# Wu-sm/Adversarial-Attacks-on-GAN-based-Image-Fusion

Measured on AMD Instinct MI355X. Metric: attacked images/sec, PGD-20 L∞ ε=8/255 at 256², 1/2/4/8 MI355X, higher is better.
Workload: dtype f32; 1 GPU; PGD-20 L∞ eps=8/255 alpha=2/255 at 256², 128 images/GPU (BASELINE config #4 per-GPU share), RCCL all-gather of outputs when N>1; encoder=e4e, norm=linf, images_per_gpu=128, global_batch=128, size=256, pgd_steps=20, parallelism=dp1, dist_world_size=1, output_in_eps_ball_and_finite=True, fp32_arithmetic=fp32

## Files before the change

adversarial-attacks-on-gan-based-image-fusion_amd/csrc/conv_halo_x6.hip:

```cpp
#include <type_traits>

#include "conv_common.h"
#include "halo_epilogue.h"

namespace mia {

#ifdef MIA_STAMPS
__device__ unsigned long long g_x6_stamps[4][24];
#endif

template <int BN_, int TPS_ = 1>
struct HaloX6 {
  static constexpr int PH = 16, PW = 16, NW = 8, NT = 64 * NW;
  static constexpr int WN = BN_ == 128 ? 2 : 1, WM = NW / WN, FM = 16 / WM, FN = 4;
  static constexpr int BM = PH * PW, BN = BN_, BK = 32;
  static constexpr int HSIDE = PW + 2, HROWS = (PH + 2) * HSIDE;
  static constexpr int HPIECES = (HROWS + 7) / 8;
  static constexpr int HBUF = HPIECES * 1024;
  static constexpr int LROWB = 64, LBUF = HROWS * LROWB;
  static constexpr int TPS = TPS_, NG = (9 + TPS - 1) / TPS;
  static constexpr int BHM = BN * ROWB, BL = BN * LROWB, BSTAGE1 = BHM + BL;
  static constexpr int BSTAGE = TPS * BSTAGE1;
  static constexpr int BWAVES = 4, HWAVES = 4;
  static constexpr int B_HM_INS = BN / 8 / BWAVES;
// ... 480 lines not shown
    atomicAdd(g + 6, (unsigned long long)nk);
    atomicAdd(g + 7, st_wb);
  }
  if (wid == 4 && lane == 0) atomicAdd(&g_x6_stamps[(BN_ == 128 ? 1 : 0) + (PRO ? 2 : 0)][8], st_wb);
  if ((wid == 0 || wid == 4) && lane == 0) {
    unsigned long long* g = g_x6_stamps[(BN_ == 128 ? 1 : 0) + (PRO ? 2 : 0)] + (wid ? 13 : 9);
    atomicAdd(g + 0, st_rd);
    atomicAdd(g + 1, st_m0);
    atomicAdd(g + 2, st_arr);
    atomicAdd(g + 3, st_rel);
  }
#endif
}

template <int BN_, bool PRO, int EPI, bool EARLY, bool PRIO = false, bool UNR = false,
          int TPS = 1, int STG = 0>
static int launch_x6_e(ConvK& k, hipStream_t st) {
  MIA_CONV_PATH("halo_x6", EPI);
  typedef HaloX6<BN_, TPS> TL;
  k.nbn = (k.a.Cout + TL::BN - 1) / TL::BN;
  k.nblk = k.a.N * (k.a.H / TL::PH) * (k.a.W / TL::PW) * k.nbn;
  size_t lds = TL::LDS;
  lds = std::max(lds, (size_t)TL::EROWS * TL::ES * 4);
  lds = std::max(lds, (size_t)TL::NW * TL::BN * 4);
  auto fn = conv_halo_x6_kernel<BN_, PRO, EPI, EARLY, PRIO, UNR, TPS, STG>;
  if (const int rc = ensure_dyn_lds((const void*)fn, 160 * 1024); rc != MIA_OK) return rc;
  k.prered = EPI >= 0 && (EPI & epi::CSUM);
  const int H = k.a.H, W = k.a.W;
  const int nslots = EPI >= 0    ? halo_red_slots(H, W, TL::FM, TL::WM, k.prered)
                     : EPI == -1 ? halo_red_slots(H, W, TL::FM, TL::WM, false)
                                 : (H / TL::PH) * (W / TL::PW);
  RedQ r;
  int rc = conv_red_begin(k, r, nslots, st);
  if (rc != MIA_OK) return rc;
  hipLaunchKernelGGL(fn, dim3(k.nblk), dim3(TL::NT), lds, st, k);
  rc = check_launch("conv_halo_x6");
  return rc != MIA_OK ? rc : red_finish(r, st);
}

constexpr bool x6_stagger_wins(bool pro, int epi) {
#ifdef MIA_X6_STAGGER_ALL
  return MIA_X6_STAGGER_ALL != 0;
#else
  (void)epi;
  return !pro;
#endif
}

template <int BN_, bool PRO, int EPI>
static int launch_x6_(ConvK& k, hipStream_t st) {
  if constexpr (EPI >= 0) {
    const int u = tune(T_X6_UNR);
    if constexpr (BN_ == 64) {
      if (u == 2) return launch_x6_e<BN_, PRO, EPI, true, true, true, 2>(k, st);
    }
    if constexpr (BN_ == 128) {
      const int sg = tune(T_X6_STAGGER);
      if (u != 0 && (sg < 0 ? x6_stagger_wins(PRO, EPI) : sg != 0))
        return launch_x6_e<BN_, PRO, EPI, true, true, true, 1, 1>(k, st);
    }
    if (u != 0) return launch_x6_e<BN_, PRO, EPI, true, true, true>(k, st);
  }
  return launch_x6_e<BN_, PRO, EPI, true, true>(k, st);
}

struct HaloX6S {
  static constexpr int PH = 8, PW = 16, NW = 4, NT = 64 * NW;
  static constexpr int WN = 1, WM = 4, FM = 2, FN = 4;
  static constexpr int BM = PH * PW, BN = 64, BK = 32;
  static constexpr int HSIDE = PW + 2, HROWS = (PH + 2) * HSIDE;
  static constexpr int HPIECES = (HROWS + 7) / 8;
  static constexpr int HBUF = HPIECES * 1024;
  static constexpr int LROWB = 64, LBUF = HROWS * LROWB;
  static constexpr int BHM = BN * ROWB, BL = BN * LROWB, BSTAGE = BHM + BL;
  static constexpr int B_HM_INS = BN / 8 / NW, B_L_INS = BN / 16 / NW;
  static constexpr int H_INS = (HPIECES + NW - 1) / NW;
  static constexpr int EROWS = 128, ES = BN + 4;
  static constexpr int LDS = HBUF + LBUF + 2 * BSTAGE;
  static_assert(WM * FM * 16 == BM && WN * FN * 16 == BN, "");
  static_assert(B_HM_INS * 8 * NW == BN && B_L_INS * 16 * NW == BN, "");
  static_assert(LDS <= 80 * 1024, "two blocks per CU");
};

template <bool PRO, int EPI>
__global__ __launch_bounds__(HaloX6S::NT, 2) void conv_halo_x6s_kernel(const ConvK k) {
  static_assert(EPI >= 0, "the specialised register epilogues only");
  typedef HaloX6S TL;
  constexpr int FM = TL::FM, FN = TL::FN, NT = TL::NT, BN = TL::BN, BK = TL::BK;
  constexpr int HSIDE = TL::HSIDE, HROWS = TL::HROWS, HPIECES = TL::HPIECES;
  constexpr int H_INS = TL::H_INS, B_HM_INS = TL::B_HM_INS, B_L_INS = TL::B_L_INS;
  constexpr int BSTAGE = TL::BSTAGE;

  extern __shared__ __attribute__((aligned(16))) char smem[];
  char* const hbuf = smem;
  char* const lbuf = smem + TL::HBUF;
  char* const bring = lbuf + TL::LBUF;

  const mia_conv_args& p = k.a;
  const int tid = threadIdx.x, lane = tid & 63;
  const int wid = __builtin_amdgcn_readfirstlane(tid >> 6);
  const int wm = wid, wn = 0;
  const ConvGroup G = k.g[0];
  const int H = p.H, W = p.W, Cin = p.Cin, Cout = p.Cout, Kpad = G.kpad;
  const int bl = xcd_remap(blockIdx.x, k.nblk);
  const int mt = bl / k.nbn, n0 = (bl % k.nbn) * BN;
  const int ptx = W / TL::PW, pty = H / TL::PH;
  const int x0 = (mt % ptx) * TL::PW;
  const int y0 = ((mt / ptx) % pty) * TL::PH;
  const int n = mt / (ptx * pty);

  const float* __restrict__ X = (const float*)p.x;
  const unsigned* __restrict__ Whm = (const unsigned*)G.w_split;
  const __bf16* __restrict__ Wl = (const __bf16*)(Whm + (size_t)Cout * Kpad);
  const char* zero = (const char*)g_zero16;

  const char* wsrc[B_HM_INS + B_L_INS];
#pragma unroll
  for (int j = 0; j < B_HM_INS + B_L_INS; ++j) {
    if (j < B_HM_INS) {
      const int row = (wid * B_HM_INS + j) * 8 + (lane >> 3);
      const int c = min(n0 + row, Cout - 1);
      wsrc[j] = (const char*)(Whm + (size_t)c * Kpad + ((lane & 7) ^ fsw(row)) * 4);
    } else {
      const int row = (wid * B_L_INS + j - B_HM_INS) * 16 + (lane >> 2);
      const int c = min(n0 + row, Cout - 1);
      wsrc[j] = (const char*)(Wl + (size_t)c * Kpad + ((lane & 3) ^ (lsw(row) >> 1)) * 8);
    }
  }
  const char* hsrc[H_INS];
#pragma unroll
  for (int j = 0; j < H_INS; ++j) {
    hsrc[j] = nullptr;
    const int hr = (wid + TL::NW * j) * 8 + (lane >> 3);
    const int hy = hr / HSIDE, hx = hr - (hr / HSIDE) * HSIDE;
    const int y = y0 + hy - 1, x = x0 + hx - 1;
    if (hr < HROWS && y >= 0 && y < H && x >= 0 && x < W)
      hsrc[j] = (const char*)(X + ((size_t)(n * H + y) * W + x) * Cin + ((lane & 7) ^ fsw(hr)) * 4);
  }
  const int ncb = Cin / BK, nk = 9 * ncb;

  auto issue_b = [&](int s, int st) {
    const int cb = s / 9, t = s - (s / 9) * 9;
    const size_t koff = (size_t)t * Cin + cb * BK;
    char* dst = bring + st * BSTAGE;
#pragma unroll
    for (int j = 0; j < B_HM_INS; ++j)
      __builtin_amdgcn_global_load_lds((gptr_t)(wsrc[j] + koff * 4),
                                       (lptr_t)(dst + (wid * B_HM_INS + j) * 1024), 16, 0, 0);
#pragma unroll
    for (int j = 0; j < B_L_INS; ++j)
      __builtin_amdgcn_global_load_lds((gptr_t)(wsrc[B_HM_INS + j] + koff * 2),
                                       (lptr_t)(dst + TL::BHM + (wid * B_L_INS + j) * 1024), 16,
                                       0, 0);
  };
  auto issue_halo = [&](int cb) {
#pragma unroll
    for (int j = 0; j < H_INS; ++j) {
      if (wid + TL::NW * j >= HPIECES) break;
      const char* a = hsrc[j] ? hsrc[j] + (size_t)cb * BK * 4 : zero;
      __builtin_amdgcn_global_load_lds((gptr_t)a, (lptr_t)(hbuf + (wid + TL::NW * j) * 1024), 16,
                                       0, 0);
    }
  };
  const bool lrelu_in = p.act_in == MIA_ACT_LRELU_S2;
  auto convert = [&](int cb) {
    for (int c = tid; c < HROWS * 8; c += NT) {
      const int hr = c >> 3, pc = c & 7, lc = pc ^ fsw(hr);
      f32x4 v = *(const f32x4*)(hbuf + hr * ROWB + pc * 16);
      if constexpr (PRO) {
        const float mul = lrelu_in ? SQRT2 : 1.f;
        f32x4 s4 = {1.f, 1.f, 1.f, 1.f};
        if (p.in_scale) s4 = *(const f32x4*)(p.in_scale + (size_t)n * Cin + cb * BK + lc * 4);
#pragma unroll
        for (int e = 0; e < 4; ++e) {
          float f = v[e];
          if (lrelu_in) f = fmaxf(f, 0.2f * f);
          v[e] = f * (s4[e] * mul);
        }
      }
      u32x4 hm;
      u32x2 lo;
      split_quad(v, hm, lo);
      *(u32x4*)(hbuf + hr * ROWB + pc * 16) = hm;
      *(u32x2*)(lbuf + hr * TL::LROWB + ((lc ^ lsw(hr)) << 3)) = lo;
    }
  };

  issue_halo(0);
  issue_b(0, 0);
  asm volatile("s_waitcnt vmcnt(0)" ::: "memory");
  __syncthreads();
  convert(0);
  __syncthreads();

  f32x4 acc[FM][FN];
#pragma unroll
  for (int i = 0; i < FM; ++i)
#pragma unroll
    for (int j = 0; j < FN; ++j) acc[i][j] = f32x4{0.f, 0.f, 0.f, 0.f};

  const int frow = lane & 15, fq = lane >> 4;
  int oh[FM + 2][3], ol[FM + 2][3];
#pragma unroll
  for (int q = 0; q < FM + 2; ++q)
#pragma unroll
    for (int c = 0; c < 3; ++c) {
      const int hr = (wm * FM + q) * HSIDE + frow + c;
      int vh = hr * ROWB + ((fq ^ fsw(hr)) << 4), vl = hr * TL::LROWB + ((fq ^ lsw(hr)) << 3);
      asm volatile("" : "+v"(vh), "+v"(vl));
      oh[q][c] = vh;
      ol[q][c] = vl;
    }
  int st = 0;
  for (int cb = 0; cb < ncb; ++cb) {
#pragma unroll
    for (int t = 0; t < 9; ++t) {
      const int s = cb * 9 + t;
      int x1 = 64, x2 = 32;
      asm volatile("" : "+s"(x1), "+s"(x2));
      const int dy = t / 3, dx = t % 3;
      const char* sb = bring + st * BSTAGE;
      if (s + 1 < nk) issue_b(s + 1, st ^ 1);
#pragma unroll
      for (int h = 0; h < 2; ++h) {
        const int ch = h * 4 + fq;
        u32x4 ahm[FM], bhm[FN];
        u32x2 al[FM], blo[FN];
#pragma unroll
        for (int i = 0; i < FM; ++i) {
          ahm[i] = *(const u32x4*)(hbuf + (h ? oh[i + dy][dx] ^ x1 : oh[i + dy][dx]));
          al[i] = *(const u32x2*)(lbuf + (h ? ol[i + dy][dx] ^ x2 : ol[i + dy][dx]));
        }
#pragma unroll
        for (int j = 0; j < FN; ++j) {
          const int row = 16 * j + frow;
          bhm[j] = *(const u32x4*)(sb + row * ROWB + ((ch ^ fsw(row)) << 4));
          blo[j] = *(const u32x2*)(sb + TL::BHM + row * TL::LROWB + ((ch ^ lsw(row)) << 3));
        }
        __builtin_amdgcn_s_setprio(1);
#pragma unroll
        for (int i = 0; i < FM; ++i)
#pragma unroll
          for (int j = 0; j < FN; ++j)
            acc[i][j] = mfma_x6(bhm[j], blo[j], ahm[i], al[i], acc[i][j]);
        __builtin_amdgcn_s_setprio(0);
      }
      asm volatile("s_waitcnt vmcnt(0)" ::: "memory");
      lds_handoff();
      __builtin_amdgcn_sched_barrier(0);
      st ^= 1;
    }
    if (cb + 1 < ncb) {
      issue_halo(cb + 1);
      asm volatile("s_waitcnt vmcnt(0)" ::: "memory");
      __syncthreads();
      convert(cb + 1);
      __syncthreads();
    }
  }
  halo_epilogue_f<float, TL, EPI>(k, acc, n, y0, x0, n0, wm, wn, lane, -1, -1, nullptr,
                                  k.prered ? (float*)smem : nullptr, TL::WM, TL::BN);
}

template <bool PRO, int EPI>
static int launch_x6s_(ConvK& k, hipStream_t st) {
  MIA_CONV_PATH("halo_x6", EPI);
  typedef HaloX6S TL;
  k.nbn = (k.a.Cout + TL::BN - 1) / TL::BN;
  k.nblk = k.a.N * (k.a.H / TL::PH) * (k.a.W / TL::PW) * k.nbn;
  size_t lds = TL::LDS;
  lds = std::max(lds, (size_t)TL::EROWS * TL::ES * 4);
  lds = std::max(lds, (size_t)TL::NW * TL::BN * 4);
  auto fn = conv_halo_x6s_kernel<PRO, EPI>;
  if (const int rc = ensure_dyn_lds((const void*)fn, 80 * 1024); rc != MIA_OK) return rc;
  k.prered = (EPI & epi::CSUM);
  const int nslots = halo_red_slots(k.a.H, k.a.W, TL::FM, TL::WM, k.prered);
  RedQ r;
  int rc = conv_red_begin(k, r, nslots, st);
  if (rc != MIA_OK) return rc;
  hipLaunchKernelGGL(fn, dim3(k.nblk), dim3(TL::NT), lds, st, k);
  rc = check_launch("conv_halo_x6s");
  return rc != MIA_OK ? rc : red_finish(r, st);
}

constexpr int X6S_NONE = 1;
static int launch_x6s(ConvK& k, hipStream_t st, bool pro) {
  using namespace epi;
  const int f = epi_mask(k);
  if (pro) {
    if (f == (OSC | NOISE | BIAS | LRELU)) return launch_x6s_<true, OSC | NOISE | BIAS | LRELU>(k, st);
    return X6S_NONE;
  }
  switch (f) {
    case 0: return launch_x6s_<false, 0>(k, st);
    case BIAS: return launch_x6s_<false, BIAS>(k, st);
    case BIAS | RELU: return launch_x6s_<false, BIAS | RELU>(k, st);
    case PRELU: return launch_x6s_<false, PRELU>(k, st);
    case MASK: return launch_x6s_<false, MASK>(k, st);
    case TAP: return launch_x6s_<false, TAP>(k, st);
    case TAP | MASK: return launch_x6s_<false, TAP | MASK>(k, st);
    case ACC: return launch_x6s_<false, ACC>(k, st);
    case MASK | MSL: return launch_x6s_<false, MASK | MSL>(k, st);
    default: return X6S_NONE;
  }
}

template <int BN_, bool PRO>
static int launch_x6_spec(ConvK& k, hipStream_t st) {
  using namespace epi;
  const int f = epi_mask(k);
  if constexpr (PRO) {
    if (f == (OSC | NOISE | BIAS | LRELU))
      return launch_x6_<BN_, PRO, OSC | NOISE | BIAS | LRELU>(k, st);
  } else if constexpr (BN_ == 64) {
    switch (f) {
      case 0: return launch_x6_<BN_, PRO, 0>(k, st);
      case BIAS: return launch_x6_<BN_, PRO, BIAS>(k, st);
      case BIAS | RELU: return launch_x6_<BN_, PRO, BIAS | RELU>(k, st);
      case PRELU: return launch_x6_<BN_, PRO, PRELU>(k, st);
      case MASK: return launch_x6_<BN_, PRO, MASK>(k, st);
      case TAP: return launch_x6_<BN_, PRO, TAP>(k, st);
      case ACC: return launch_x6_<BN_, PRO, ACC>(k, st);
      case MASK | MSL: return launch_x6_<BN_, PRO, MASK | MSL>(k, st);
      default: break;
    }
  } else {
    switch (f) {
      case 0: return launch_x6_<BN_, PRO, 0>(k, st);
      case BIAS: return launch_x6_<BN_, PRO, BIAS>(k, st);
      case BIAS | RELU: return launch_x6_<BN_, PRO, BIAS | RELU>(k, st);
      case PRELU: return launch_x6_<BN_, PRO, PRELU>(k, st);
      case MASK: return launch_x6_<BN_, PRO, MASK>(k, st);
      case TAP: return launch_x6_<BN_, PRO, TAP>(k, st);
      case ACC: return launch_x6_<BN_, PRO, ACC>(k, st);
      case MASK | MSL: return launch_x6_<BN_, PRO, MASK | MSL>(k, st);
      case OSC | SDOT: return launch_x6_<BN_, PRO, OSC | SDOT>(k, st);
      case OSC | SDOT | BAB: return launch_x6_<BN_, PRO, OSC | SDOT | BAB>(k, st);
      default: break;
    }
  }
  return launch_x6_<BN_, PRO, -1>(k, st);
}

bool conv_halo_x6_eligible(const ConvK& k, int dtype) {
#ifdef MIA_F32_NATIVE
  (void)k;
  (void)dtype;
  return false;
#endif
  if (tune(T_CONV_X6) == 0) return false;
  const mia_conv_args& a = k.a;
  const ConvGroup& G = k.g[0];
  return dtype == MIA_F32 && G.w_split != nullptr && k.ng == 1 && k.stride == 1 && G.kh == 3 &&
         G.kw == 3 && G.pad_y == 1 && G.pad_x == 1 && G.ho == a.H && G.wo == a.W && G.ay == 1 &&
         G.ax == 1 && G.by == 0 && G.bx == 0 && !a.shuffle_out && a.H % 16 == 0 &&
         a.W % 16 == 0 && a.Cin % 32 == 0 && k.HT == a.H && k.WT == a.W &&
         a.Cout >= 64;
}

#ifdef MIA_STAMPS
extern "C" int mia_debug_x6_stamps(unsigned long long* host, int reset) {
  if (hipMemcpyFromSymbol(host, HIP_SYMBOL(g_x6_stamps), sizeof(g_x6_stamps)) != hipSuccess)
    return 1;
  if (reset) {
    static const unsigned long long zero[4][24] = {};
// ... 39 lines not shown
```

adversarial-attacks-on-gan-based-image-fusion_amd/csrc/conv_upconv.hip:

```cpp
#include "conv_common.h"

namespace mia {

template <int BN_>
struct HaloUpT {
  static constexpr int PH = 8, PW = 16, NW = 4, NT = 256;
  static constexpr int WN = BN_ == 64 ? 2 : 1, WM = NW / WN, FM = PH / WM, FN = 2;
  static constexpr int BN = WN * FN * 16;
  static constexpr int HSIDE = PW + 1, HROWS = (PH + 1) * HSIDE;
  static constexpr int HPIECES = (HROWS + 7) / 8;
  static constexpr int HBUF = HPIECES * 8 * ROWB;
  static constexpr int BROWS = 2 * BN, BSTAGE = BROWS * ROWB;
  static constexpr int BWAVES = 2, HWAVES = 2;
  static constexpr int B_INS = BROWS / (8 * BWAVES);
  static constexpr int H_INS = (HPIECES + HWAVES - 1) / HWAVES;
  static constexpr int HPS = (H_INS + 3) / 4;
  static constexpr int NSTEP = 5, STAGES = 2;
  static_assert(B_INS * 8 * BWAVES == BROWS && H_INS * HWAVES == HPIECES, "");
  static_assert(WM * FM == PH && WN * FN * 16 == BN_, "");
};
typedef HaloUpT<64> HaloUp;

__device__ __forceinline__ constexpr int up_jy(int st) { return st == 3 || st == 4 ? 1 : 0; }
__device__ __forceinline__ constexpr int up_jx(int st) { return st == 2 || st == 4 ? 1 : 0; }
// ... 537 lines not shown
#pragma unroll
            for (int j = 0; j < FN; ++j)
              acc[ph][i][j] = mfma_x6(bhm[j], blo[j], ahm[i], al[i], acc[ph][i][j]);
          if constexpr (PRIO) __builtin_amdgcn_s_setprio(0);
        }
        if (!EARLY && h == 0 && !bwave && st < 4 && cb + 1 < ncb) {
          __builtin_amdgcn_sched_barrier(0);
#pragma unroll
          for (int q = 0; q < HPS; ++q) {
            const int j = st * HPS + q;
            if (j < H_INS && hw + HWAVES * j < HPIECES) issue_h(cb + 1, j, (cb + 1) & 1);
          }
          __builtin_amdgcn_sched_barrier(0);
        }
      }
      if (bwave || st == TL::NSTEP - 1) asm volatile("s_waitcnt vmcnt(0)" ::: "memory");
      __builtin_amdgcn_s_waitcnt(0xc07f);
      __builtin_amdgcn_s_barrier();
      __builtin_amdgcn_sched_barrier(0);
      if (st == TL::NSTEP - 1 && cb + 1 < ncb) {
        convert(cb + 1);
        __syncthreads();
      }
    }
  }

  const int frow = lane & 15, fq = lane >> 4;
  float* __restrict__ Y = (float*)k.t;
  const int TS = DG ? 2 * R : 2 * R + 1;
  float msl[FN][4];
#pragma unroll
  for (int j = 0; j < FN; ++j)
#pragma unroll
    for (int e = 0; e < 4; ++e)
      msl[j][e] = k.mask_slope ? k.mask_slope[n0 + wn * FN * 16 + 16 * j + 4 * fq + e] : 0.f;
#pragma unroll
  for (int ph = 0; ph < 4; ++ph) {
    const int py = ph >> 1, px = ph & 1;
#pragma unroll
    for (int i = 0; i < FM; ++i) {
      const int ty = 2 * (y0 + wm * FM + i) + (DG ? 1 - py : py);
      const int tx = 2 * (x0 + frow) + (DG ? 1 - px : px);
#pragma unroll
      for (int j = 0; j < FN; ++j) {
        const int c = n0 + wn * FN * 16 + 16 * j + 4 * fq;
        const size_t o = ((size_t)(n * TS + ty) * TS + tx) * Cout + c;
        f32x4 v = acc[ph][i][j];
        if (DG && k.mask_a) {
          const f32x4 m = *(const f32x4*)((const float*)k.mask_a + o);
#pragma unroll
          for (int e = 0; e < 4; ++e) v[e] = m[e] > 0.f ? v[e] : msl[j][e] * v[e];
        }
        if (DG && k.accumulate) {
          const f32x4 a = *(const f32x4*)(Y + o);
#pragma unroll
          for (int e = 0; e < 4; ++e) v[e] += a[e];
        }
        *(f32x4*)(Y + o) = v;
      }
    }
  }
}

struct DgX6S {
  static constexpr int PH = 8, PW = 16, NW = 4, NT = 64 * NW;
  static constexpr int WM = 4, WN = 1, FM = 2, FN = 4;
  static constexpr int BN = WN * FN * 16, BK = 32;
  static constexpr int HSIDE = PW + 1, HROWS = (PH + 1) * HSIDE;
  static constexpr int HPIECES = (HROWS + 7) / 8;
  static constexpr int HBUF = HPIECES * 1024;
  static constexpr int LROWB = 64, LBUF = HROWS * LROWB;
  static constexpr int BROWS = 2 * BN;
  static constexpr int BHM = BROWS * ROWB, BSTAGE = BHM + BROWS * LROWB;
  static constexpr int B_HM_INS = BROWS / 8 / NW;
  static constexpr int B_L_INS = BROWS / 16 / NW;
  static constexpr int H_INS = (HPIECES + NW - 1) / NW;
  static constexpr int NSTEP = 5;
  static constexpr int LDS = HBUF + LBUF + 2 * BSTAGE;
  static_assert(WM * FM == PH && WN * FN * 16 == BN, "");
  static_assert(B_HM_INS * 8 * NW == BROWS && B_L_INS * 16 * NW == BROWS, "");
  static_assert(LDS <= 80 * 1024, "two blocks per CU");
};

template <bool DG, bool PRO>
__global__ __launch_bounds__(DgX6S::NT, 2) void upconv_x6s_kernel(const UpK k) {
  typedef DgX6S TL;
  constexpr int FM = TL::FM, FN = TL::FN, WN = TL::WN, BN = TL::BN, BK = TL::BK, NT = TL::NT;
  constexpr int HSIDE = TL::HSIDE, HROWS = TL::HROWS, HPIECES = TL::HPIECES;
  constexpr int H_INS = TL::H_INS, BSTAGE = TL::BSTAGE;
  constexpr int B_HM_INS = TL::B_HM_INS, B_L_INS = TL::B_L_INS;

  extern __shared__ __attribute__((aligned(16))) char smem[];
  char* const hbuf = smem;
  char* const lbuf = smem + TL::HBUF;
  char* const bring = lbuf + TL::LBUF;

  const int tid = threadIdx.x, lane = tid & 63;
  const int wid = __builtin_amdgcn_readfirstlane(tid >> 6);
  const int wm = wid / WN, wn = wid % WN;
  const int R = k.R, Cin = k.Cin, Cout = k.Cout;
  const int bl = xcd_remap(blockIdx.x, k.nblk);
  const int mt = bl / k.nbn, n0 = (bl % k.nbn) * BN;
  const int ptx = R / TL::PW, pty = R / TL::PH;
  const int x0 = (mt % ptx) * TL::PW;
  const int y0 = ((mt / ptx) % pty) * TL::PH;
  const int n = mt / (ptx * pty);
  const int ncb = Cin / BK, nk = TL::NSTEP * ncb;
  const int csrc = k.cin_src, cbs = csrc / BK;
  const char* Whm = (const char*)k.w_split;
  const char* Wl = Whm + (size_t)nk * 2 * Cout * ROWB;
  const size_t hm_step = (size_t)2 * Cout * ROWB, l_step = (size_t)2 * Cout * TL::LROWB;
  const char* zero = (const char*)g_zero16;

  int woff[B_HM_INS + B_L_INS], hoff[H_INS];
#pragma unroll
  for (int j = 0; j < B_HM_INS + B_L_INS; ++j) {
    if (j < B_HM_INS) {
      const int row = (wid * B_HM_INS + j) * 8 + (lane >> 3);
      const int slot = row / BN, c = n0 + row % BN;
      woff[j] = (slot * Cout + c) * ROWB + ((lane & 7) ^ fsw(row)) * 16;
    } else {
      const int row = (wid * B_L_INS + j - B_HM_INS) * 16 + (lane >> 2);
      const int slot = row / BN, c = n0 + row % BN;
      woff[j] = (slot * Cout + c) * TL::LROWB + ((lane & 3) ^ (lsw(row) >> 1)) * 16;
    }
  }
#pragma unroll
  for (int j = 0; j < H_INS; ++j) {
    hoff[j] = -1;
    const int hr = (wid + TL::NW * j) * 8 + (lane >> 3);
    const int hy = hr / HSIDE, hx = hr - (hr / HSIDE) * HSIDE;
    const int y = y0 + hy - (DG ? 0 : 1), x = x0 + hx - (DG ? 0 : 1);
    if (hr < HROWS && y >= 0 && y < R && x >= 0 && x < R)
      hoff[j] = ((n * R + y) * R + x) * csrc + ((lane & 7) ^ fsw(hr)) * 4;
  }
  auto opaque = [](int v) __attribute__((always_inline)) {
    asm volatile("" : "+v"(v));
    return v;
  };
  auto issue_b = [&](int s, int stg) {
    char* dst = bring + stg * BSTAGE;
    const char* hm = Whm + s * hm_step;
    const char* lo = Wl + s * l_step;
#pragma unroll
    for (int j = 0; j < B_HM_INS; ++j)
      __builtin_amdgcn_global_load_lds((gptr_t)(hm + opaque(woff[j])),
                                       (lptr_t)(dst + (wid * B_HM_INS + j) * 1024), 16, 0, 0);
#pragma unroll
    for (int j = 0; j < B_L_INS; ++j)
      __builtin_amdgcn_global_load_lds((gptr_t)(lo + opaque(woff[B_HM_INS + j])),
                                       (lptr_t)(dst + TL::BHM + (wid * B_L_INS + j) * 1024), 16,
                                       0, 0);
  };
  auto issue_halo = [&](int cb) {
    const int sc = cb / cbs;
    const float* xb = (const float*)up_src(k, sc) + (cb - sc * cbs) * BK;
#pragma unroll
    for (int j = 0; j < H_INS; ++j) {
      if (wid + TL::NW * j >= HPIECES) break;
      const int o = opaque(hoff[j]);
      const char* a = o >= 0 ? (const char*)(xb + o) : zero;
      __builtin_amdgcn_global_load_lds((gptr_t)a, (lptr_t)(hbuf + (wid + TL::NW * j) * 1024), 16,
                                       0, 0);
    }
  };
  const bool lrelu_in = k.act_in == MIA_ACT_LRELU_S2;
  auto convert = [&](int cb) {
    for (int c = tid; c < HROWS * 8; c += NT) {
      const int hr = c >> 3, pc = c & 7, lc = pc ^ fsw(hr);
      f32x4 v = *(const f32x4*)(hbuf + hr * ROWB + pc * 16);
      if constexpr (PRO) {
        const float mul = lrelu_in ? SQRT2 : 1.f;
        f32x4 s4 = {1.f, 1.f, 1.f, 1.f};
        if (k.style) s4 = *(const f32x4*)(k.style + (size_t)n * Cin + cb * BK + lc * 4);
#pragma unroll
        for (int e = 0; e < 4; ++e) {
          float f = v[e];
          if (lrelu_in) f = fmaxf(f, 0.2f * f);
          v[e] = f * (s4[e] * mul);
        }
      }
      u32x4 hm;
      u32x2 lo;
      split_quad(v, hm, lo);
      *(u32x4*)(hbuf + hr * ROWB + pc * 16) = hm;
      *(u32x2*)(lbuf + hr * TL::LROWB + ((lc ^ lsw(hr)) << 3)) = lo;
    }
  };

  issue_halo(0);
  issue_b(0, 0);
  asm volatile("s_waitcnt vmcnt(0)" ::: "memory");
  __syncthreads();
  convert(0);
  __syncthreads();

  f32x4 acc[4][FM][FN];
#pragma unroll
  for (int q = 0; q < 4; ++q)
#pragma unroll
    for (int i = 0; i < FM; ++i)
#pragma unroll
      for (int j = 0; j < FN; ++j) acc[q][i][j] = f32x4{0.f, 0.f, 0.f, 0.f};

  for (int cb = 0; cb < ncb; ++cb) {
#pragma unroll
    for (int st = 0; st < TL::NSTEP; ++st) {
      const int ln = opaque(lane);
      const int frow = ln & 15, fq = ln >> 4;
      const int s = cb * TL::NSTEP + st;
      const char* sb = bring + (s & 1) * BSTAGE;
      if (s + 1 < nk) issue_b(s + 1, (s & 1) ^ 1);
      const int jy = up_jy(st), jx = up_jx(st);
#pragma unroll
      for (int h = 0; h < 2; ++h) {
        const int ch = h * 4 + fq;
        u32x4 ahm[FM];
        u32x2 al[FM];
#pragma unroll
        for (int i = 0; i < FM; ++i) {
          const int hr = DG ? (wm * FM + i + jy) * HSIDE + frow + jx
                            : (wm * FM + i + 1 - jy) * HSIDE + frow + 1 - jx;
          ahm[i] = *(const u32x4*)(hbuf + hr * ROWB + ((ch ^ fsw(hr)) << 4));
          al[i] = *(const u32x2*)(lbuf + hr * TL::LROWB + ((ch ^ lsw(hr)) << 3));
        }
#pragma unroll
        for (int slot = 0; slot < 2; ++slot) {
          const int ph = up_phase(st, slot);
          if (ph < 0) continue;
          u32x4 bhm[FN];
          u32x2 blo[FN];
#pragma unroll
          for (int j = 0; j < FN; ++j) {
            const int row = slot * BN + wn * FN * 16 + 16 * j + frow;
            bhm[j] = *(const u32x4*)(sb + row * ROWB + ((ch ^ fsw(row)) << 4));
            blo[j] = *(const u32x2*)(sb + TL::BHM + row * TL::LROWB + ((ch ^ lsw(row)) << 3));
          }
#pragma unroll
          for (int i = 0; i < FM; ++i)
#pragma unroll
            for (int j = 0; j < FN; ++j)
              acc[ph][i][j] = mfma_x6(bhm[j], blo[j], ahm[i], al[i], acc[ph][i][j]);
        }
      }
      asm volatile("s_waitcnt vmcnt(0)" ::: "memory");
      lds_handoff();
      __builtin_amdgcn_sched_barrier(0);
    }
    if (cb + 1 < ncb) {
      issue_halo(cb + 1);
      asm volatile("s_waitcnt vmcnt(0)" ::: "memory");
      __syncthreads();
      convert(cb + 1);
      __syncthreads();
    }
  }

  const int frow = lane & 15, fq = lane >> 4;
  float* __restrict__ Y = (float*)k.t;
  const int TS = DG ? 2 * R : 2 * R + 1;
  float msl[FN][4];
#pragma unroll
  for (int j = 0; j < FN; ++j)
#pragma unroll
    for (int e = 0; e < 4; ++e)
      msl[j][e] = k.mask_slope ? k.mask_slope[n0 + wn * FN * 16 + 16 * j + 4 * fq + e] : 0.f;
#pragma unroll
  for (int ph = 0; ph < 4; ++ph) {
    const int py = ph >> 1, px = ph & 1;
#pragma unroll
    for (int i = 0; i < FM; ++i) {
      const int ty = 2 * (y0 + wm * FM + i) + (DG ? 1 - py : py);
      const int tx = 2 * (x0 + frow) + (DG ? 1 - px : px);
#pragma unroll
      for (int j = 0; j < FN; ++j) {
        const int c = n0 + wn * FN * 16 + 16 * j + 4 * fq;
        const size_t o = ((size_t)(n * TS + ty) * TS + tx) * Cout + c;
        f32x4 v = acc[ph][i][j];
        if (DG && k.mask_a) {
          const f32x4 m = *(const f32x4*)((const float*)k.mask_a + o);
#pragma unroll
          for (int e = 0; e < 4; ++e) v[e] = m[e] > 0.f ? v[e] : msl[j][e] * v[e];
        }
        if (DG && k.accumulate) {
          const f32x4 a = *(const f32x4*)(Y + o);
#pragma unroll
          for (int e = 0; e < 4; ++e) v[e] += a[e];
        }
        *(f32x4*)(Y + o) = v;
      }
    }
  }
}

template <bool DG, bool PRO>
static int launch_upconv_x6s(UpK& k, hipStream_t st) {
  typedef DgX6S TL;
  set_conv_path(DG ? "s2dg_x6s" : "upconv_x6s");
  k.nbn = k.Cout / TL::BN;
  k.nblk = k.N * (k.R / TL::PH) * (k.R / TL::PW) * k.nbn;
  auto fn = upconv_x6s_kernel<DG, PRO>;
  if (const int rc = ensure_dyn_lds((const void*)fn, 80 * 1024); rc != MIA_OK) return rc;
  hipLaunchKernelGGL(fn, dim3(k.nblk), dim3(TL::NT), TL::LDS, st, k);
  return check_launch("upconv_x6s");
}

template <bool DG, bool PRO, bool EARLY, bool PRIO>
static int launch_upconv_x6_e(UpK& k, hipStream_t st) {
  typedef DgX6 TL;
  set_conv_path(DG ? "s2dg_x6" : "upconv_x6");
  k.nbn = k.Cout / TL::BN;
  k.nblk = k.N * (k.R / TL::PH) * (k.R / TL::PW) * k.nbn;
  auto fn = upconv_x6_kernel<DG, PRO, EARLY, PRIO>;
  if (const int rc = ensure_dyn_lds((const void*)fn, 160 * 1024); rc != MIA_OK) return rc;
  hipLaunchKernelGGL(fn, dim3(k.nblk), dim3(TL::NT), TL::LDS, st, k);
  return check_launch("upconv_x6");
}

template <bool DG, bool PRO>
static int launch_upconv_x6(UpK& k, hipStream_t st) {
  if (DG && tune(T_UPCONV_X6S) != 0 && k.Cin <= 512) return launch_upconv_x6s<DG, PRO>(k, st);
  return launch_upconv_x6_e<DG, PRO, true, false>(k, st);
}

static bool upconv_x6_ok(const UpK& k, int dtype) {
#ifdef MIA_F32_NATIVE
  (void)k;
  (void)dtype;
  return false;
#else
  if (tune(T_UPCONV_X6) == 0) return false;
  return dtype == MIA_F32 && k.w_split && k.R % DgX6::PH == 0 && k.Cout % DgX6::BN == 0 &&
         k.Cin % DgX6::BK == 0;
#endif
}

static bool s2dg_x6_ok(const UpK& k, int dtype) {
#ifdef MIA_F32_NATIVE
  (void)k;
  (void)dtype;
  return false;
#else
  if (tune(T_S2DG_X6) == 0) return false;
  return dtype == MIA_F32 && k.w_split && k.R % DgX6::PH == 0 && k.Cout % DgX6::BN == 0 &&
         k.cin_src % DgX6::BK == 0;
#endif
}

bool s2_dgrad_halo_eligible(int dtype, int R, int Cg, int Cx) {
  if (tune(T_S2DG_HALO) == 0) return false;
  (void)dtype;
  return R % 16 == 0 && Cg % 64 == 0 && Cx % HaloUp::BN == 0 &&
         (int64_t)4 * R * R < (1LL << 31);
}

}

using namespace mia;

extern "C" int mia_conv_s2_dgrad_halo_multi(const void* const* g, int ng, const void* w_halo,
                                            const void* w_split, void* gx, int N, int R, int Cg,
                                            int Cx, const void* mask_a, const float* mask_slope,
                                            int accumulate, int dtype, void* stream) {
  MIA_CHECK_ARG(g && ng >= 1 && ng <= UP_MAX_SRC && w_halo && gx && N > 0, "bad args");
  for (int i = 0; i < ng; ++i) MIA_CHECK_ARG(g[i], "null source tensor");
  MIA_CHECK_ARG(s2_dgrad_halo_eligible(dtype, R, Cg, Cx),
                "needs R % 16 == 0, Cg % 64 == 0, Cx % 64 == 0 "
                "(use mia_conv2d phase groups otherwise)");
  MIA_CHECK_ARG((int64_t)N * R * R * Cg < (1LL << 31), "input too large for 32-bit offsets");
  UpK k = {};
  k.x = g[0]; k.w = w_halo; k.t = gx; k.mask_a = mask_a; k.mask_slope = mask_slope;
  k.N = N; k.R = R; k.Cin = ng * Cg; k.Cout = Cx; k.accumulate = accumulate;
  for (int i = 0; i < ng; ++i) k.xs[i] = g[i];
  k.cin_src = Cg;
  k.w_split = w_split;
  if (s2dg_x6_ok(k, dtype)) return launch_upconv_x6<true, false>(k, (hipStream_t)stream);
  MIA_DISPATCH_DTYPE(dtype, T, return launch_upconv_halo<T, false, true>(k, (hipStream_t)stream));
  return set_error("s2_dgrad_halo: unknown dtype");
}


extern "C" int mia_conv_s2_dgrad_halo(const void* g, const void* w_halo, void* gx, int N, int R,
                                      int Cg, int Cx, const void* mask_a, const float* mask_slope,
                                      int accumulate, int dtype, void* stream) {
  const void* gs[1] = {g};
  return mia_conv_s2_dgrad_halo_multi(gs, 1, w_halo, nullptr, gx, N, R, Cg, Cx, mask_a,
                                      mask_slope, accumulate, dtype, stream);
// ... 2 lines not shown
```

adversarial-attacks-on-gan-based-image-fusion_amd/csrc/mia_common.h:

```cpp
#pragma once
#include <hip/hip_runtime.h>
#include <stdint.h>
#include <string>

#include "../../include/miattack.h"

namespace mia {

typedef __attribute__((ext_vector_type(4))) float f32x4;
typedef __attribute__((ext_vector_type(8))) _Float16 f16x8;
typedef __attribute__((ext_vector_type(8))) __bf16 bf16x8;

template <typename T> struct Vec;
template <> struct Vec<float> { typedef f32x4 type; static constexpr int N = 4; };
template <> struct Vec<_Float16> { typedef f16x8 type; static constexpr int N = 8; };
template <> struct Vec<__bf16> { typedef bf16x8 type; static constexpr int N = 8; };

__device__ __forceinline__ float to_f(float v) { return v; }
__device__ __forceinline__ float to_f(_Float16 v) { return (float)v; }
__device__ __forceinline__ float to_f(__bf16 v) { return (float)v; }
template <typename T> __device__ __forceinline__ T from_f(float v);
template <> __device__ __forceinline__ float from_f<float>(float v) { return v; }
template <> __device__ __forceinline__ _Float16 from_f<_Float16>(float v) { return (_Float16)v; }
template <> __device__ __forceinline__ __bf16 from_f<__bf16>(float v) { return (__bf16)v; }

constexpr float SQRT2 = 1.41421356237309504880f;

__device__ __forceinline__ float lrelu_s2(float v) { return (v > 0.f ? v : 0.2f * v) * SQRT2; }
__device__ __forceinline__ float lrelu_s2_grad(float pre) { return pre > 0.f ? SQRT2 : 0.2f * SQRT2; }
__device__ __forceinline__ float lrelu_s2_inv_grad(float pre) {
  return pre > 0.f ? 0.70710678118654752f : 3.5355339059327376f;
}

#define MIA_DPP(v, ctrl) \
  __builtin_bit_cast(float, __builtin_amdgcn_mov_dpp(__builtin_bit_cast(int, (v)), (ctrl), 0xf, 0xf, false))
__device__ __forceinline__ void lds_handoff() {
  asm volatile("s_waitcnt lgkmcnt(0)\n\ts_barrier" ::: "memory");
}

__device__ __forceinline__ float row16_sum(float v) {
  v += MIA_DPP(v, 0xB1);
  v += MIA_DPP(v, 0x4E);
  v += MIA_DPP(v, 0x141);
  v += MIA_DPP(v, 0x140);
  return v;
}

__device__ __forceinline__ float wave_sum(float v) {
#pragma unroll
  for (int o = 32; o > 0; o >>= 1) v += __shfl_xor(v, o, 64);
  return v;
}

int set_error(const std::string& msg);
int check_launch(const char* what);

int device_cu_count();
int ensure_dyn_lds(const void* fn, int bytes);
int max_blocks_per_cu(const void* fn, int threads, size_t dyn_lds);

enum TuneKey {
  T_CONV_HALO,
  T_CONV_X6,
  T_HALO_EPI,
  T_X6_UNR,
  T_CONV_THIN,
  T_CONV_THIN32,
  T_CONV_WRES,
  T_CONV_REGEPI,
  T_CONV_SMALLTILE,
  T_S2DG_X6,
  T_S2DG_HALO,
  T_UPCONV_X6,
  T_UPCONV_HALO,
  T_CONV_WRES32,
  T_HALO_C64,
  T_X6_64S,
  T_UPCONV_X6S,
  T_CONV_WRES128,
  T_X6_STAGGER,
  T_NKEYS
};
int tune(TuneKey key);

struct RedQ {
  float* dst[3];
  float* part;
  int nslots, count;
};
float* red_scratch(hipStream_t st, size_t bytes);
int red_begin(RedQ& r, float* d0, float* d1, float* d2, int nslots, int count, hipStream_t st,
              bool zero = false);
int red_finish(const RedQ& r, hipStream_t st);

__device__ __forceinline__ void red_store(float* part, int nslots, int count, int q, int slot,
                                          int i, float v) {
  part[((size_t)q * nslots + slot) * count + i] = v;
}

}

#define MIA_DISPATCH_DTYPE(dtype, T, ...)                                   \
  switch (dtype) {                                                          \
    case MIA_F32: { typedef float T; __VA_ARGS__; break; }                  \
    case MIA_F16: { typedef _Float16 T; __VA_ARGS__; break; }               \
    case MIA_BF16: { typedef __bf16 T; __VA_ARGS__; break; }                \
    default: return mia::set_error("unsupported dtype");                    \
  }

#define MIA_CHECK_ARG(cond, msg) \
  do { if (!(cond)) return mia::set_error(std::string(__func__) + ": " + (msg)); } while (0)
```

adversarial-attacks-on-gan-based-image-fusion_amd/csrc/reduce.hip:

```cpp
#include <algorithm>
#include <cstdlib>
#include <cstring>
#include <mutex>
#include <unordered_map>
#include <vector>

#include "mia_common.h"

namespace mia {

namespace {
struct Scratch {
  float* p = nullptr;
  size_t bytes = 0;
};
std::mutex g_mu;
std::unordered_map<hipStream_t, Scratch> g_scratch;
}

namespace {
struct TuneDef {
  const char* name;
  int value;
};
TuneDef g_tune[T_NKEYS] = {
    {"MIA_CONV_HALO", 1}, {"MIA_CONV_X6", 1},       {"MIA_HALO_EPI", 1},    {"MIA_X6_UNR", 2},
    {"MIA_CONV_THIN", 1}, {"MIA_CONV_THIN32", 1},   {"MIA_CONV_WRES", 1},
    {"MIA_CONV_REGEPI", 1},   {"MIA_CONV_SMALLTILE", 512},
    {"MIA_S2DG_X6", 1},   {"MIA_S2DG_HALO", 1},     {"MIA_UPCONV_X6", 1},   {"MIA_UPCONV_HALO", 1},
    {"MIA_CONV_WRES32", 1},
    {"MIA_HALO_C64", 1},  {"MIA_X6_64S", 1},
    {"MIA_UPCONV_X6S", 1}, {"MIA_CONV_WRES128", 1}, {"MIA_X6_STAGGER", -1}};
std::once_flag g_tune_once;
void tune_init() {
  for (auto& d : g_tune) {
    if (&d == &g_tune[T_X6_STAGGER]) continue;
    const char* e = getenv(d.name);
    if (e && *e) d.value = atoi(e);
  }
}
}

int tune(TuneKey key) {
  std::call_once(g_tune_once, tune_init);
  return g_tune[key].value;
}

namespace {
std::mutex g_dev_mu;
std::unordered_map<int, int> g_ncu;
std::unordered_map<const void*, std::vector<int>> g_lds_set;
int current_device() {
  int dev = 0;
  (void)hipGetDevice(&dev);
  return dev;
}
}

int device_cu_count() {
  const int dev = current_device();
  std::lock_guard<std::mutex> lock(g_dev_mu);
  auto it = g_ncu.find(dev);
  if (it != g_ncu.end()) return it->second;
  int ncu = 0;
  if (hipDeviceGetAttribute(&ncu, hipDeviceAttributeMultiprocessorCount, dev) != hipSuccess ||
      ncu <= 0)
    ncu = 256;
  g_ncu[dev] = ncu;
  return ncu;
}

int ensure_dyn_lds(const void* fn, int bytes) {
  const int dev = current_device();
  std::lock_guard<std::mutex> lock(g_dev_mu);
  std::vector<int>& done = g_lds_set[fn];
  if (std::find(done.begin(), done.end(), dev) != done.end()) return MIA_OK;
  if (hipFuncSetAttribute(fn, hipFuncAttributeMaxDynamicSharedMemorySize, bytes) != hipSuccess)
    return set_error("hipFuncSetAttribute(MaxDynamicSharedMemorySize) failed");
  done.push_back(dev);
  return MIA_OK;
}

int max_blocks_per_cu(const void* fn, int threads, size_t dyn_lds) {
  static std::unordered_map<const void*, std::unordered_map<int, int>> cache;
  const int dev = current_device();
  std::lock_guard<std::mutex> lock(g_dev_mu);
  auto& per_dev = cache[fn];
  auto it = per_dev.find(dev);
  if (it != per_dev.end()) return it->second;
  int occ = 0;
  if (hipOccupancyMaxActiveBlocksPerMultiprocessor(&occ, fn, threads, dyn_lds) != hipSuccess ||
      occ < 1)
    occ = 1;
  per_dev[dev] = occ;
  return occ;
}

float* red_scratch(hipStream_t st, size_t bytes) {
  std::lock_guard<std::mutex> lock(g_mu);
  Scratch& s = g_scratch[st];
  if (s.bytes >= bytes) return s.p;
  if (s.p) {
    if (hipStreamSynchronize(st) != hipSuccess || hipFree(s.p) != hipSuccess) return nullptr;
    s.p = nullptr;
    s.bytes = 0;
  }
  size_t want = bytes < (1u << 20) ? (1u << 20) : bytes;
  want = want + want / 4;
  void* p = nullptr;
  if (hipMalloc(&p, want) != hipSuccess) return nullptr;
  s.p = (float*)p;
  s.bytes = want;
  return s.p;
}

constexpr int RED_CHUNK = 64;
static inline int red_nchunks(int nslots) { return nslots <= 2 * RED_CHUNK ? 1 : (nslots + RED_CHUNK - 1) / RED_CHUNK; }

int red_begin(RedQ& r, float* d0, float* d1, float* d2, int nslots, int count, hipStream_t st,
// ... 143 lines not shown
```

Baseline: 17.58 attacked images/s.

## Prefetch next channel-block halo into registers during last k-steps of x6s convs

In the small-tile x6 halo conv and the upconv x6s kernels, the next channel block's halo tile is now loaded from global memory into registers a couple of k-steps before the current block ends. The loads overlap with the remaining MFMA work, then are converted and written to LDS. This replaces the serial issue, wait, sync and convert sequence at block boundaries and removes one barrier. The cost is extra VGPRs for the prefetch buffer, which may hurt occupancy at two blocks per CU, and hardcoded vmcnt wait counts. The path is on by default and cannot be disabled through the environment.

```diff
diff --git a/adversarial-attacks-on-gan-based-image-fusion_amd/csrc/conv_halo_x6.hip b/adversarial-attacks-on-gan-based-image-fusion_amd/csrc/conv_halo_x6.hip
--- a/adversarial-attacks-on-gan-based-image-fusion_amd/csrc/conv_halo_x6.hip
+++ b/adversarial-attacks-on-gan-based-image-fusion_amd/csrc/conv_halo_x6.hip
@@ -586,9 +586,12 @@
   static_assert(LDS <= 80 * 1024, "two blocks per CU");
 };
 
-template <bool PRO, int EPI>
+constexpr int X6S_PFD = 2;
+
+template <bool PRO, int EPI, bool PF>
 __global__ __launch_bounds__(HaloX6S::NT, 2) void conv_halo_x6s_kernel(const ConvK k) {
   static_assert(EPI >= 0, "the specialised register epilogues only");
+  static_assert(X6S_PFD >= 1 && X6S_PFD <= 8, "issued inside the block it follows");
   typedef HaloX6S TL;
   constexpr int FM = TL::FM, FN = TL::FN, NT = TL::NT, BN = TL::BN, BK = TL::BK;
   constexpr int HSIDE = TL::HSIDE, HROWS = TL::HROWS, HPIECES = TL::HPIECES;
@@ -690,6 +693,39 @@
     }
   };
 
+  f32x4 pf[H_INS];
+  auto load_halo = [&](int cb) {
+#pragma unroll
+    for (int j = 0; j < H_INS; ++j) {
+      const char* a = hsrc[j] ? hsrc[j] + (size_t)cb * BK * 4 : zero;
+      pf[j] = *(const f32x4*)a;
+    }
+  };
+  auto convert_regs = [&](int cb) {
+#pragma unroll
+    for (int j = 0; j < H_INS; ++j) {
+      const int hr = (wid + TL::NW * j) * 8 + (lane >> 3), pc = lane & 7, lc = pc ^ fsw(hr);
+      if (hr >= HROWS) continue;
+      f32x4 v = pf[j];
+      if constexpr (PRO) {
+        const float mul = lrelu_in ? SQRT2 : 1.f;
+        f32x4 s4 = {1.f, 1.f, 1.f, 1.f};
+        if (p.in_scale) s4 = *(const f32x4*)(p.in_scale + (size_t)n * Cin + cb * BK + lc * 4);
+#pragma unroll
+        for (int e = 0; e < 4; ++e) {
+          float f = v[e];
+          if (lrelu_in) f = fmaxf(f, 0.2f * f);
+          v[e] = f * (s4[e] * mul);
+        }
+      }
+      u32x4 hm;
+      u32x2 lo;
+      split_quad(v, hm, lo);
+      *(u32x4*)(hbuf + hr * ROWB + pc * 16) = hm;
+      *(u32x2*)(lbuf + hr * TL::LROWB + ((lc ^ lsw(hr)) << 3)) = lo;
+    }
+  };
+
   issue_halo(0);
   issue_b(0, 0);
   asm volatile("s_waitcnt vmcnt(0)" ::: "memory");
@@ -716,15 +752,14 @@
       ol[q][c] = vl;
     }
   int st = 0;
-  for (int cb = 0; cb < ncb; ++cb) {
-#pragma unroll
-    for (int t = 0; t < 9; ++t) {
+  auto kstep = [&](int cb, int t, bool pf_step) __attribute__((always_inline)) {
       const int s = cb * 9 + t;
       int x1 = 64, x2 = 32;
       asm volatile("" : "+s"(x1), "+s"(x2));
       const int dy = t / 3, dx = t % 3;
       const char* sb = bring + st * BSTAGE;
       if (s + 1 < nk) issue_b(s + 1, st ^ 1);
+      if (pf_step) load_halo(cb + 1);
 #pragma unroll
       for (int h = 0; h < 2; ++h) {
         const int ch = h * 4 + fq;
@@ -749,12 +784,32 @@
             acc[i][j] = mfma_x6(bhm[j], blo[j], ahm[i], al[i], acc[i][j]);
         __builtin_amdgcn_s_setprio(0);
       }
-      asm volatile("s_waitcnt vmcnt(0)" ::: "memory");
+      if (pf_step) {
+        static_assert(H_INS == 6, "the wait count below");
+        asm volatile("s_waitcnt vmcnt(6)" ::: "memory");
+      } else {
+        asm volatile("s_waitcnt vmcnt(0)" ::: "memory");
+      }
       lds_handoff();
       __builtin_amdgcn_sched_barrier(0);
       st ^= 1;
-    }
-    if (cb + 1 < ncb) {
+  };
+  for (int cb = 0; cb < ncb; ++cb) {
+    constexpr int TP = PF ? 9 - X6S_PFD : 9;
+#pragma unroll
+    for (int t = 0; t < TP; ++t) kstep(cb, t, false);
+    if constexpr (PF) {
+      if (cb + 1 < ncb) {
+#pragma unroll
+        for (int t = TP; t < 9; ++t) kstep(cb, t, t == TP);
+        convert_regs(cb + 1);
+        lds_handoff();
+        __builtin_amdgcn_sched_barrier(0);
+      } else {
+#pragma unroll
+        for (int t = TP; t < 9; ++t) kstep(cb, t, false);
+      }
+    } else if (cb + 1 < ncb) {
       issue_halo(cb + 1);
       asm volatile("s_waitcnt vmcnt(0)" ::: "memory");
       __syncthreads();
@@ -766,16 +821,16 @@
                                   k.prered ? (float*)smem : nullptr, TL::WM, TL::BN);
 }
 
-template <bool PRO, int EPI>
-static int launch_x6s_(ConvK& k, hipStream_t st) {
-  MIA_CONV_PATH("halo_x6", EPI);
+template <bool PRO, int EPI, bool PF>
+static int launch_x6s_pf(ConvK& k, hipStream_t st) {
+  MIA_CONV_PATH("halo_x6s", EPI);
   typedef HaloX6S TL;
   k.nbn = (k.a.Cout + TL::BN - 1) / TL::BN;
   k.nblk = k.a.N * (k.a.H / TL::PH) * (k.a.W / TL::PW) * k.nbn;
   size_t lds = TL::LDS;
   lds = std::max(lds, (size_t)TL::EROWS * TL::ES * 4);
   lds = std::max(lds, (size_t)TL::NW * TL::BN * 4);
-  auto fn = conv_halo_x6s_kernel<PRO, EPI>;
+  auto fn = conv_halo_x6s_kernel<PRO, EPI, PF>;
   if (const int rc = ensure_dyn_lds((const void*)fn, 80 * 1024); rc != MIA_OK) return rc;
   k.prered = (EPI & epi::CSUM);
   const int nslots = halo_red_slots(k.a.H, k.a.W, TL::FM, TL::WM, k.prered);
@@ -785,6 +840,12 @@
   hipLaunchKernelGGL(fn, dim3(k.nblk), dim3(TL::NT), lds, st, k);
   rc = check_launch("conv_halo_x6s");
   return rc != MIA_OK ? rc : red_finish(r, st);
+}
+
+template <bool PRO, int EPI>
+static int launch_x6s_(ConvK& k, hipStream_t st) {
+  return tune(T_X6S_PREFETCH) != 0 ? launch_x6s_pf<PRO, EPI, true>(k, st)
+                                   : launch_x6s_pf<PRO, EPI, false>(k, st);
 }
 
 constexpr int X6S_NONE = 1;
diff --git a/adversarial-attacks-on-gan-based-image-fusion_amd/csrc/conv_upconv.hip b/adversarial-attacks-on-gan-based-image-fusion_amd/csrc/conv_upconv.hip
--- a/adversarial-attacks-on-gan-based-image-fusion_amd/csrc/conv_upconv.hip
+++ b/adversarial-attacks-on-gan-based-image-fusion_amd/csrc/conv_upconv.hip
@@ -643,8 +643,11 @@
   static_assert(LDS <= 80 * 1024, "two blocks per CU");
 };
 
-template <bool DG, bool PRO>
+constexpr int DGS_PFD = 2;
+
+template <bool DG, bool PRO, bool PF>
 __global__ __launch_bounds__(DgX6S::NT, 2) void upconv_x6s_kernel(const UpK k) {
+  static_assert(DGS_PFD >= 1 && DGS_PFD < DgX6S::NSTEP, "issued inside the block it follows");
   typedef DgX6S TL;
   constexpr int FM = TL::FM, FN = TL::FN, WN = TL::WN, BN = TL::BN, BK = TL::BK, NT = TL::NT;
   constexpr int HSIDE = TL::HSIDE, HROWS = TL::HROWS, HPIECES = TL::HPIECES;
@@ -749,6 +752,43 @@
     }
   };
 
+  static_assert(TL::NW * H_INS == HPIECES, "the same load count in every wave");
+  f32x4 pf[H_INS];
+  auto load_halo = [&](int cb) {
+    const int sc = cb / cbs;
+    const float* xb = (const float*)up_src(k, sc) + (cb - sc * cbs) * BK;
+#pragma unroll
+    for (int j = 0; j < H_INS; ++j) {
+      const int o = opaque(hoff[j]);
+      const char* a = o >= 0 ? (const char*)(xb + o) : zero;
+      pf[j] = *(const f32x4*)a;
+    }
+  };
+  auto convert_regs = [&](int cb) {
+#pragma unroll
+    for (int j = 0; j < H_INS; ++j) {
+      const int hr = (wid + TL::NW * j) * 8 + (lane >> 3), pc = lane & 7, lc = pc ^ fsw(hr);
+      if (hr >= HROWS) continue;
+      f32x4 v = pf[j];
+      if constexpr (PRO) {
+        const float mul = lrelu_in ? SQRT2 : 1.f;
+        f32x4 s4 = {1.f, 1.f, 1.f, 1.f};
+        if (k.style) s4 = *(const f32x4*)(k.style + (size_t)n * Cin + cb * BK + lc * 4);
+#pragma unroll
+        for (int e = 0; e < 4; ++e) {
+          float f = v[e];
+          if (lrelu_in) f = fmaxf(f, 0.2f * f);
+          v[e] = f * (s4[e] * mul);
+        }
+      }
+      u32x4 hm;
+      u32x2 lo;
+      split_quad(v, hm, lo);
+      *(u32x4*)(hbuf + hr * ROWB + pc * 16) = hm;
+      *(u32x2*)(lbuf + hr * TL::LROWB + ((lc ^ lsw(hr)) << 3)) = lo;
+    }
+  };
+
   issue_halo(0);
   issue_b(0, 0);
   asm volatile("s_waitcnt vmcnt(0)" ::: "memory");
@@ -771,7 +811,9 @@
       const int frow = ln & 15, fq = ln >> 4;
       const int s = cb * TL::NSTEP + st;
       const char* sb = bring + (s & 1) * BSTAGE;
+      const bool pf_step = PF && st == TL::NSTEP - DGS_PFD && cb + 1 < ncb;
       if (s + 1 < nk) issue_b(s + 1, (s & 1) ^ 1);
+      if (pf_step) load_halo(cb + 1);
       const int jy = up_jy(st), jx = up_jx(st);
 #pragma unroll
       for (int h = 0; h < 2; ++h) {
@@ -804,16 +846,27 @@
               acc[ph][i][j] = mfma_x6(bhm[j], blo[j], ahm[i], al[i], acc[ph][i][j]);
         }
       }
-      asm volatile("s_waitcnt vmcnt(0)" ::: "memory");
+      if (pf_step) {
+        static_assert(H_INS == 5, "the wait count below");
+        asm volatile("s_waitcnt vmcnt(5)" ::: "memory");
+      } else {
+        asm volatile("s_waitcnt vmcnt(0)" ::: "memory");
+      }
       lds_handoff();
       __builtin_amdgcn_sched_barrier(0);
     }
     if (cb + 1 < ncb) {
-      issue_halo(cb + 1);
-      asm volatile("s_waitcnt vmcnt(0)" ::: "memory");
-      __syncthreads();
-      convert(cb + 1);
-      __syncthreads();
+      if constexpr (PF) {
+        convert_regs(cb + 1);
+        lds_handoff();
+        __builtin_amdgcn_sched_barrier(0);
+      } else {
+        issue_halo(cb + 1);
+        asm volatile("s_waitcnt vmcnt(0)" ::: "memory");
+        __syncthreads();
+        convert(cb + 1);
+        __syncthreads();
+      }
     }
   }
 
@@ -854,16 +907,22 @@
   }
 }
 
-template <bool DG, bool PRO>
-static int launch_upconv_x6s(UpK& k, hipStream_t st) {
+template <bool DG, bool PRO, bool PF>
+static int launch_upconv_x6s_pf(UpK& k, hipStream_t st) {
   typedef DgX6S TL;
   set_conv_path(DG ? "s2dg_x6s" : "upconv_x6s");
   k.nbn = k.Cout / TL::BN;
   k.nblk = k.N * (k.R / TL::PH) * (k.R / TL::PW) * k.nbn;
-  auto fn = upconv_x6s_kernel<DG, PRO>;
+  auto fn = upconv_x6s_kernel<DG, PRO, PF>;
   if (const int rc = ensure_dyn_lds((const void*)fn, 80 * 1024); rc != MIA_OK) return rc;
   hipLaunchKernelGGL(fn, dim3(k.nblk), dim3(TL::NT), TL::LDS, st, k);
   return check_launch("upconv_x6s");
+}
+
+template <bool DG, bool PRO>
+static int launch_upconv_x6s(UpK& k, hipStream_t st) {
+  return tune(T_X6S_PREFETCH) != 0 ? launch_upconv_x6s_pf<DG, PRO, true>(k, st)
+                                   : launch_upconv_x6s_pf<DG, PRO, false>(k, st);
 }
 
 template <bool DG, bool PRO, bool EARLY, bool PRIO>
diff --git a/adversarial-attacks-on-gan-based-image-fusion_amd/csrc/mia_common.h b/adversarial-attacks-on-gan-based-image-fusion_amd/csrc/mia_common.h
--- a/adversarial-attacks-on-gan-based-image-fusion_amd/csrc/mia_common.h
+++ b/adversarial-attacks-on-gan-based-image-fusion_amd/csrc/mia_common.h
@@ -79,6 +79,7 @@
   T_UPCONV_X6S,
   T_CONV_WRES128,
   T_X6_STAGGER,
+  T_X6S_PREFETCH,
   T_NKEYS
 };
 int tune(TuneKey key);
diff --git a/adversarial-attacks-on-gan-based-image-fusion_amd/csrc/reduce.hip b/adversarial-attacks-on-gan-based-image-fusion_amd/csrc/reduce.hip
--- a/adversarial-attacks-on-gan-based-image-fusion_amd/csrc/reduce.hip
+++ b/adversarial-attacks-on-gan-based-image-fusion_amd/csrc/reduce.hip
@@ -30,11 +30,12 @@
     {"MIA_S2DG_X6", 1},   {"MIA_S2DG_HALO", 1},     {"MIA_UPCONV_X6", 1},   {"MIA_UPCONV_HALO", 1},
     {"MIA_CONV_WRES32", 1},
     {"MIA_HALO_C64", 1},  {"MIA_X6_64S", 1},
-    {"MIA_UPCONV_X6S", 1}, {"MIA_CONV_WRES128", 1}, {"MIA_X6_STAGGER", -1}};
+    {"MIA_UPCONV_X6S", 1}, {"MIA_CONV_WRES128", 1}, {"MIA_X6_STAGGER", -1},
+    {"MIA_X6S_PREFETCH", 1}};
 std::once_flag g_tune_once;
 void tune_init() {
   for (auto& d : g_tune) {
-    if (&d == &g_tune[T_X6_STAGGER]) continue;
+    if (&d == &g_tune[T_X6_STAGGER] || &d == &g_tune[T_X6S_PREFETCH]) continue;
     const char* e = getenv(d.name);
     if (e && *e) d.value = atoi(e);
   }
```

Measured after the change: 17.62 attacked images/s (median of 6 runs). Within noise of the previous version (+0.2%).
